# mgdesaix/WGSassign

Measured on AMD Instinct MI355X. Metric: EM SNP-updates/s (per-population update, n_call=100), higher is better.
Workload: dtype f64; 1 GPU; 1 GPU(s), SNP-sharded: synthetic Beagle 10000000 SNPs x 1000 ind, K=10, EM sweep; mode=exact, snps_per_gpu=10000000, gl_bytes_per_gpu=80000000000, comm_native_rccl=False, step=wgs_em_fit iteration (enqueued ahead of the host)

## Files before the change

### wgsassign_amd/csrc/codes.hip

```cpp
#include <chrono>
#include <cstdlib>
#include <cstring>

#include "common.h"

static double now_s() { return std::chrono::duration<double>(std::chrono::steady_clock::now().time_since_epoch()).count(); }

static void pool_join(wgs_beagle *b)
{
    if (b->pool_thread) {
        b->pool_thread->join();
        delete b->pool_thread;
        b->pool_thread = nullptr;
    }
}

static int pool_adopt(wgs_beagle *b)
{
    const int st = b->pool_state.load();
    if (st == 0) return b->pool ? 1 : -1;
    if (st == 1) return 0;
    pool_join(b);
    b->pool_state.store(0);
    if (st < 0) return -1;
// ... 53 lines not shown
    (void)hipFree(b->pool);
    b->pool = nullptr;
    b->pool_bytes = 0;
    return pool_request(b, want, want_small, grace_ms);
}

extern "C" int wgs_beagle_codes_wait(wgs_beagle *b, double *alloc_ms)
{
    WGS_REQUIRE(b, "null argument");
    if (alloc_ms) *alloc_ms = 0.0;
    if (b->pool_state.load() == 0) return 0;
    HIP_TRY(hipSetDevice(b->ctx->device));
    while (b->pool_state.load() == 1) std::this_thread::sleep_for(std::chrono::microseconds(100));
    (void)pool_adopt(b);
    if (alloc_ms) *alloc_ms = b->pool_alloc_ms;
    return 0;
}

void wgs_beagle_release_pool(wgs_beagle *b)
{
    if (!b) return;
    pool_join(b);
    if (b->pool_new) (void)hipFree(b->pool_new);
    b->pool_new = nullptr;
    b->pool_state.store(0);
    if (b->pool) (void)hipFree(b->pool);
    b->pool = nullptr;
    b->pool_bytes = 0;
}

void wgs_beagle_drop_codes(wgs_beagle *b)
{
    if (!b) return;
    if (wgs_codes *c = b->codes) {
        (void)hipSetDevice(b->ctx->device);
        (void)hipStreamSynchronize(b->ctx->stream);
        delete c;
    }
    b->codes = nullptr;
    b->codes_state = 0;
    b->plan = wgs_codes_plan();
    b->direct_sweeps = 0;
    ++b->codes_generation;
}

bool codes_switched_off()
{
    const char *env = getenv("WGSASSIGN_CODES");
    return env && env[0] == '0';
}

double wgs_em_codes_saving(double classes_per_slab, double cols, int lrows)
{
    const double saves = std::max(0.0, std::min(0.6, 1.0 - 2.2 * classes_per_slab / std::max(1.0, cols)));
    if (lrows <= 24) return saves;
    const double waves = std::max(1.0, std::min(13.0, floor(160.0 * 1024.0 / ((double)lrows * 512.0))));
    return std::max(0.0, 1.0 - (1.0 - saves) * pow(13.0 / waves, 0.8));
}

static int hist_quantile(const unsigned long long *h, double share)
{
    unsigned long long total = 0, run = 0;
    for (int i = 0; i < 256; ++i) total += h[i];
    if (!total) return 0;
    const double want = share * (double)total;
    for (int i = 0; i < 256; ++i) {
        run += h[i];
        if ((double)run >= want) return i;
    }
    return 255;
}

static double hist_mean(const unsigned long long *h)
{
    unsigned long long total = 0;
    double sum = 0.0;
    for (int i = 0; i < 256; ++i) total += h[i], sum += (double)i * (double)h[i];
    return total ? sum / (double)total : 0.0;
}

const wgs_codes_plan *wgs_beagle_codes_plan(wgs_beagle *b)
{
    if (!b) return nullptr;
    wgs_codes_plan &P = b->plan;
    if (P.state != 0) return &P;
    P = wgs_codes_plan();
    P.state = -1;
    if (hipSetDevice(b->ctx->device) != hipSuccess) return &P;
    const double t0 = now_s();
    wgs_codes tmpc;
    tmpc.slabs.resize(b->n_groups);
    for (int g = 0; g < b->n_groups; ++g) tmpc.slabs[g].nquads = (b->slabs[g].ncols + 3) / 4;
    void *tmp = nullptr;
    if (wgs_ctx_workspace_b(b->ctx, sizeof(SlabCodes) * b->n_groups, &tmp)) return &P;
    tmpc.d_slabs = reinterpret_cast<SlabCodes *>(tmp);
    if (hipMemcpy(tmpc.d_slabs, tmpc.slabs.data(), sizeof(SlabCodes) * b->n_groups, hipMemcpyHostToDevice) != hipSuccess) return &P;
    unsigned long long hg[256], hl[256];
    if (launch_class_sample(b, &tmpc, 4096, hg, hl, nullptr)) {
        (void)hipGetLastError();
        return &P;
    }
    P.mean_g = hist_mean(hg);
    P.mean_l = hist_mean(hl);
    const int g999 = hist_quantile(hg, 0.999), g99 = hist_quantile(hg, 0.99);
    const char *force = getenv("WGSASSIGN_CODES_TABLE");
    P.slots = g99 <= 44 ? 64 : (g99 <= 88 ? 128 : 256);
    if (force && (atoi(force) == 64 || atoi(force) == 128 || atoi(force) == 256)) P.slots = atoi(force);
// ... 202 lines not shown
```

### wgsassign_amd/csrc/common.h

```cpp
#pragma once
#include <hip/hip_runtime.h>
#include <stdint.h>

#include <atomic>
#include <chrono>
#include <thread>
#include <vector>

#include "../../include/wgsassign_hip.h"
#include "../../include/wgsassign_hip_debug.h"
#include "em_fit_ledger.h"

void wgs_set_error(const char *fmt, ...);

#ifdef WGS_TRACE_STALLS
#include <chrono>
#include <cstdio>
struct wgs_stall_probe {
    const char *what, *file;
    int line;
    std::chrono::steady_clock::time_point t0 = std::chrono::steady_clock::now();
    ~wgs_stall_probe() {
        const double ms = std::chrono::duration<double, std::milli>(std::chrono::steady_clock::now() - t0).count();
        if (ms >= WGS_TRACE_STALLS) fprintf(stderr, "[stall] %.1f ms in %s (%s:%d)\n", ms, what, file, line);
// ... 20 lines not shown
    } while (0)

extern std::atomic<long long> g_wgs_malloc_ns;
template <typename T>
static inline hipError_t wgs_malloc(T **p, size_t bytes)
{
    const auto t0 = std::chrono::steady_clock::now();
    const hipError_t e = hipMalloc(p, bytes);
    g_wgs_malloc_ns += std::chrono::duration_cast<std::chrono::nanoseconds>(std::chrono::steady_clock::now() - t0).count();
    return e;
}

#define WGS_REQUIRE(cond, ...)          \
    do {                                \
        if (!(cond)) {                  \
            wgs_set_error(__VA_ARGS__); \
            return 2;                   \
        }                               \
    } while (0)

template <typename F>
struct ScopeFail {
    F fn;
    bool armed = true;
    explicit ScopeFail(F f) : fn(f) {}
    ~ScopeFail() { if (armed) fn(); }
    void dismiss() { armed = false; }
};
template <typename F>
ScopeFail<F> on_failure(F f) { return ScopeFail<F>(f); }

struct wgs_ctx {
    int device = 0;
    hipStream_t stream = nullptr;
    void *pinned = nullptr;
    size_t pinned_bytes = 0;
    int cus = 0;
    void *ws = nullptr;
    size_t ws_bytes = 0;
    void *ws_b = nullptr;
    size_t ws_b_bytes = 0;
    bool log_table_ready = false;
    hipEvent_t ev0 = nullptr, ev1 = nullptr;
    float last_assign_ms = 0.0f;
    bool assign_ms_pending = false;
    std::atomic<int> allocs_in_flight{0};
    struct PoolBlock {
        void *p;
        size_t bytes;
        bool used;
    };
    std::vector<PoolBlock> pool;
    int64_t dyn_lds_base = -1;
    hipEvent_t enc_ev0 = nullptr, enc_ev1 = nullptr;
};
int wgs_ctx_workspace(wgs_ctx *ctx, size_t bytes, void **out);
hipError_t wgs_pool_malloc(wgs_ctx *ctx, void **p, size_t bytes);
void wgs_pool_free(wgs_ctx *ctx, void *p);
template <typename T>
static inline hipError_t wgs_pool_malloc(wgs_ctx *ctx, T **p, size_t bytes)
{
    return wgs_pool_malloc(ctx, reinterpret_cast<void **>(p), bytes);
}

struct Slab {
    float4 *base = nullptr;
    int32_t npairs = 0;
    int32_t ncols = 0;
    std::vector<int32_t> members;
    int32_t *d_members = nullptr;
};
static inline int64_t wgs_ntiles(int64_t m) { return (m + 63) / 64; }

#ifndef WGS_ENC_SLOTS
#define WGS_ENC_SLOTS 1024
#endif
constexpr int WGS_ENC_MIN_SNPS = WGS_ENC_SLOTS / 256;
constexpr int WGS_TILE_ROWS_BYTES = 64 / WGS_ENC_MIN_SNPS;
constexpr int WGS_BATCH_ROWS_CAP = 616;
struct SlabCodes {
    uint32_t *codes = nullptr;
    uint32_t *lcodes = nullptr;
    float2 *ldict = nullptr;
    uint8_t *tile_rows = nullptr;
    int32_t nquads = 0;
    int32_t quad0 = 0;
};
struct wgs_codes {
    void *pool = nullptr;
    int32_t snps_per_wave = 16;
    int32_t drows = 0;
    int32_t lrows = 0;
    int32_t cmax = 0;
    int32_t score_batch = 16;
    int32_t rows_batch = 0;
    int32_t total_quads = 0;
    float2 *dict = nullptr;
    uint8_t *ncls = nullptr;
    std::vector<SlabCodes> slabs;
    SlabCodes *d_slabs = nullptr;
    uint4 *wave_stats = nullptr;
    int64_t bytes = 0, local_bytes = 0;
    int64_t generation = 0;
    double build_ms = 0.0, kernel_ms = 0.0, sample_ms = 0.0, alloc_ms = 0.0, alloc_wait_ms = 0.0;
    double sum_ncls = 0.0;
    int64_t rich_snps = 0;
// ... 75 lines not shown
enum { WGS_LIVE_EM = 1, WGS_LIVE_SCORE = 2 };
void wgs_live_add(void *obj, int kind, void *parent, void *parent2 = nullptr);
bool wgs_live_remove(void *obj);
void wgs_live_destroy_children(void *parent);

int64_t wgs_hook(const char *name);

struct wgs_afset {
    wgs_ctx *ctx = nullptr;
    int64_t m = 0;
    int32_t K = 0;
    float *buf = nullptr;
};


struct FitDesc {
    const float4 *slab;
    const float *f_old;
    float *f_new;
    double *ssq;
    double *ssq_part;
    float *f_new2;
    double *ssq2;
    double *ssq_part2;
    int32_t fuse;
    int32_t npairs, ncols;
    int32_t skip;
    int32_t n_eff;
    const int32_t *state;
    const uint32_t *lcodes;
    const float2 *ldict;
    const uint8_t *tile_rows;
    int32_t nquads, lrows;
};
struct ChainJob {
    const float *a, *b;
    float carry_in;
};

struct FisherDesc {
    const float4 *slab;
    const float *th;
    float *f_out, *ne_out;
    int32_t npairs, ncols;
};
int launch_fisher_pop(wgs_ctx *ctx, const FisherDesc *d_descs, int32_t n_desc, int64_t m);
int launch_fisher_ind_sites(wgs_ctx *ctx, const float4 *slab, const int32_t *d_cols, const float *th, float *d_out, int64_t m,
                            int npairs, int count);
int launch_pairwise_mean(wgs_ctx *ctx, const float *d_rows, int count, int64_t m, int64_t divide_by, const int64_t *d_leaf_lo,
                         const int32_t *d_leaf_len, int nleaf, const int32_t *d_prog, int nprog, float *d_leaf_sums, const float *d_carry,
                         float *d_means);
int launch_em_sweep(wgs_ctx *ctx, const FitDesc *d_descs, int32_t n_fits, int64_t m, int mode);
int launch_em_coded(wgs_ctx *ctx, const FitDesc *d_descs, int32_t n_fits, int64_t m, int rows);
bool em_coded_usable(wgs_ctx *ctx);
int launch_em_coded_groups(wgs_ctx *ctx, const FitDesc *d_descs, const int32_t *d_groups, int32_t n_groups, int64_t m, int rows);
int em_fits_per_group(void);
int launch_em_sweep_groups(wgs_ctx *ctx, const FitDesc *d_descs, const int32_t *d_groups, int32_t n_groups, int64_t m, int mode);
int ssq_reduce_chunks(void);
int launch_ssq_reduce(wgs_ctx *ctx, const FitDesc *d_descs, int32_t n_fits, int64_t m, double *part2, int second = 0);
int launch_em_decide(wgs_ctx *ctx, const FitDesc *d_descs, int32_t n_fits, double lo, double hi);
int launch_rcp_error(wgs_ctx *ctx, int exponent, unsigned long long *d_max_bits);
int launch_div_check(wgs_ctx *ctx, unsigned long long seed, unsigned long long per_thread, unsigned long long *d_mismatch);
int launch_fill(wgs_ctx *ctx, float *p, int64_t count, float v);
int launch_clamp(wgs_ctx *ctx, float *p, int64_t count, float lo, float hi);
int launch_rmse_chain_serial(wgs_ctx *ctx, const float *a, const float *b, int64_t m, float carry_in, float *d_out);
size_t rmse_chain_workspace_bytes(int64_t m);
int launch_rmse_chain(wgs_ctx *ctx, const float *a, const float *b, int64_t m, float carry_in, float *d_out, void *work,
                      int *d_serial);
int launch_chain_set_carry(wgs_ctx *ctx, ChainJob *d_jobs, const float *d_carry, int n_jobs);
int launch_rmse_chain_batch(wgs_ctx *ctx, const ChainJob *d_jobs, int n_jobs, int64_t m, float *d_out, void *work, int *d_serial);
int launch_em_stream_add_sums(wgs_ctx *ctx, const double *d_window, double *d_total, int n);
int launch_em_stream_add_sums_above(wgs_ctx *ctx, const double *d_window, double *d_total, const int32_t *d_from, int t, int n);
int launch_em_stream_chain_load(wgs_ctx *ctx, ChainJob *d_jobs, const int32_t *d_cell, const float *d_table, int n_jobs);
int launch_em_stream_chain_store(wgs_ctx *ctx, const float *d_out, const int32_t *d_cell, float *d_table, int n_jobs);

struct AssignArgs {
    const float4 *slab;
    const int32_t *members;
    const float *const *colptr;
    const float *const *acol;
    double *out;
    int64_t m, site0;
    int32_t npairs, ncols, K, P;
    int32_t tiles_per_wave;
};
int launch_assign(wgs_ctx *ctx, const AssignArgs &a, int kb, int mode);
struct PartsSlab {
    const float4 *slab;
    const int32_t *members;
    int32_t npairs, ncols;
    int32_t block0;
};
int launch_parts_exact(wgs_ctx *ctx, const AssignArgs &a, const PartsSlab *d_slabs, int n_slabs, int total_blocks,
                       const float *d_carry, float *d_parts);

constexpr int WGS_BLOCK_TILES = 64;
struct ScoreSlab {
    const float4 *slab;
    const int32_t *members;
    int32_t npairs, ncols;
    int32_t pair0;
    int32_t npg;
    int32_t pg0;
    int32_t col_lo, col_hi;
};
struct ScoreArgs {
    const ScoreSlab *slabs;
// ... 61 lines not shown
```

### wgsassign_amd/csrc/em_api.hip

```cpp
#include <math.h>
#include <string.h>

#include <algorithm>
#include <chrono>
#include <string>

#include "common.h"
#include "em_state.h"
#include "em_stream_checks.h"

template <class Launch> static int em_launch_sliced(size_t units, size_t per_launch, Launch launch)
{
    for (size_t off = 0; off < units; off += per_launch)
        if (launch(off, (int)std::min(per_launch, units - off))) return 1;
    return 0;
}

extern "C" {



void wgs_em_destroy(wgs_em *em)
{
    if (!em || !wgs_live_remove(em)) return;
// ... 47 lines not shown
    em->pend_cur.assign(n_fits, 0);
    em->pend_prev.assign(n_fits, 1);
    em->active.assign(n_fits, 1);
    for (int j = 0; j < n_fits; ++j) {
        const int g = fit_group[j];
        if (g < 0 || g >= b->n_groups || b->slabs[g].ncols == 0) {
            wgs_set_error("fit %d: group %d is out of range or empty", j, g);
            return 2;
        }
        int skip = -1;
        if (fit_skip && fit_skip[j] >= 0) {
            const int i = fit_skip[j];
            if (i >= b->n || b->group_of[i] != g) {
                wgs_set_error("fit %d: left-out individual %d does not belong to group %d", j, i, g);
                return 2;
            }
            skip = b->col_of[i];
        }
        em->group[j] = g;
        em->skip_local[j] = skip;
        em->n_eff[j] = b->slabs[g].ncols - (skip >= 0 ? 1 : 0);
    }
    const size_t fbytes = (size_t)n_fits * b->m * sizeof(float);
    for (int i = 0; i < 2; ++i) {
        if (wgs_malloc(&em->fbuf[i], fbytes) != hipSuccess) {
            wgs_set_error("hipMalloc of %zu bytes for EM frequencies failed", fbytes);
            return 1;
        }
    }
    HIP_TRY(wgs_malloc(&em->d_ssq, sizeof(double) * n_fits));
    HIP_TRY(wgs_malloc(&em->d_part, sizeof(double) * (size_t)n_fits * wgs_ntiles(b->m)));
    HIP_TRY(wgs_malloc(&em->d_part2, sizeof(double) * (size_t)n_fits * ssq_reduce_chunks()));
    HIP_TRY(wgs_malloc(&em->d_carry, 2 * sizeof(float)));
    HIP_TRY(wgs_malloc(&em->d_chain_work, rmse_chain_workspace_bytes(b->m)));
    HIP_TRY(hipEventCreate(&em->ev0));
    HIP_TRY(hipEventCreate(&em->ev1));
    for (int i = 0; i < 2; ++i) {
        HIP_TRY(wgs_malloc(&em->d_descs[i], sizeof(FitDesc) * n_fits));
        HIP_TRY(hipHostMalloc(&em->h_descs[i], sizeof(FitDesc) * n_fits, hipHostMallocDefault));
        HIP_TRY(wgs_malloc(&em->d_groups[i], sizeof(int32_t) * 2 * n_fits));
        HIP_TRY(hipHostMalloc(&em->h_groups[i], sizeof(int32_t) * 2 * n_fits, hipHostMallocDefault));
    }
    if (launch_fill(b->ctx, em->fbuf[0], (int64_t)n_fits * b->m, 0.25f)) return 1;
    HIP_TRY(hipStreamSynchronize(b->ctx->stream));
    guard.dismiss();
    *out = em;
    return 0;
}


static double loo_codes_saving(const wgs_codes_plan *P, double cols)
{
    if (!P || P->state <= 0 || P->lrows == 0) return 0.0;
    return 1.0 - (1.7 * P->mean_l * 29.0 + 4.0 * cols + 250.0) / (25.9 * std::max(1.0, cols));
}

struct EmCodesModel {
    double direct_ms = 0.0, saves = 0.0, build_ms = 0.0;
    bool sampled = false;
    bool codable = false;
    bool pays = false;
};
static EmCodesModel em_codes_model(wgs_beagle *b, double swept, double cols, bool shared, bool sample)
{
    EmCodesModel M;
    if (shared) {
        constexpr double LOO_MS_PER_TERM = 7.6e-10;
        M.direct_ms = swept / 8.0 * LOO_MS_PER_TERM;
    } else {
        M.direct_ms = swept / 6.0e9;
        M.saves = wgs_em_codes_saving(4.6 * pow(std::max(1.0, cols), 0.25), cols, 24);
        M.build_ms = wgs_codes_build_ms_estimate(b, 64);
        M.codable = true;
        if (!sample) return M;
    }
    const wgs_codes_plan *P = wgs_beagle_codes_plan(b);
    M.sampled = true;
    M.codable = P && P->state > 0 && P->lrows > 0;
    if (!M.codable) {
        M.saves = 0.0;
        return M;
    }
    M.saves = shared ? std::max(0.0, loo_codes_saving(P, cols)) : wgs_em_codes_saving(P->mean_l, cols, P->lrows);
    M.build_ms = wgs_codes_build_ms_estimate(b, P->slots);
    return M;
}

static EmCodesModel em_codes_decide(wgs_beagle *b, double swept, double cols, bool shared, double ahead)
{
    const EmCodesModel T = em_codes_model(b, swept, cols, false, false);
    if (!shared && ahead * T.saves * T.direct_ms <= T.build_ms) return T;
    EmCodesModel M = em_codes_model(b, swept, cols, shared, true);
    M.pays = M.codable && ahead * M.saves * M.direct_ms > M.build_ms;
    return M;
}

static int env_int(const char *name, int unset) { const char *v = getenv(name); return v ? atoi(v) : unset; }

struct EmSwitches {
    bool codes = !codes_switched_off();
    bool loo_codes = env_int("WGSASSIGN_LOO_CODES", 1) != 0;
    int codes_min = env_int("WGSASSIGN_EM_CODES_MIN", 28);
    bool sweeps_set = getenv("WGSASSIGN_EM_CODES_SWEEPS") != nullptr;
    int sweeps_min = env_int("WGSASSIGN_EM_CODES_SWEEPS", 0);
    bool fuse = env_int("WGSASSIGN_EM_FUSE", 2) >= 2;
};

// ... 45 lines not shown
    const int64_t ntiles = wgs_ntiles(em->b->m);
    if (wgs_malloc(&em->fbuf[2], fbytes) != hipSuccess || wgs_malloc(&em->d_part_b, sizeof(double) * (size_t)em->n_fits * ntiles) != hipSuccess) {
        (void)hipGetLastError();
        if (em->fbuf[2]) (void)hipFree(em->fbuf[2]);
        em->fbuf[2] = nullptr;
        return false;
    }
    return true;
}

struct EmSweepPlan {
    std::vector<int32_t> order;
    bool shared = false;
    int fits_per_group = 1;
    wgs_codes *codes = nullptr;
    bool can_fuse = false;
    bool fusing = false;
    const std::vector<int32_t> *may_fuse = nullptr;
};

static EmSweepPlan em_plan_sweep(wgs_em *em, const std::vector<int32_t> &list, int sweeps_ahead, const std::vector<int32_t> *may_fuse,
                                 bool fuse_agreed, const EmSwitches &sw)
{
    wgs_beagle *b = em->b;
    EmSweepPlan p;
    double swept = 0.0, cols = 0.0;
    int fewest = INT32_MAX;
    std::vector<char> seen(b->n_groups, 0);
    for (int j : list) {
        const int g = em->group[j], ncols = b->slabs[g].ncols;
        p.shared = p.shared || seen[g];
        seen[g] = 1;
        swept += 8.0 * (double)ncols * (double)b->m;
        cols += (double)ncols;
        fewest = std::min(fewest, ncols);
    }
    cols /= (double)list.size();
    p.order = list;
    if (p.shared) std::stable_sort(p.order.begin(), p.order.end(), [&](int32_t x, int32_t y) { return em->group[x] < em->group[y]; });
    const bool worth = em->mode == WGS_MODE_EXACT && sw.codes && (!p.shared || sw.loo_codes) && fewest >= sw.codes_min &&
                       (!p.shared || sw.sweeps_set || loo_codes_saving(wgs_beagle_codes_plan(b), cols) > 0.03);
    const bool build = worth && em_codes_pay(em, swept, cols, sweeps_ahead, p.shared, sw);
    {
        WGS_STALL_SCOPE("wgs_beagle_codes from the sweep");
        p.codes = worth ? wgs_beagle_codes(b, build, false) : nullptr;
        if (p.codes && p.codes->lrows == 0 && p.codes->local_skipped && build) {
            const wgs_codes_plan keep = b->plan;
            wgs_beagle_drop_codes(b);
            b->plan = keep;
            p.codes = wgs_beagle_codes(b, true, false);
        }
    }
    WGS_STALL_SCOPE("the sweep's plan");
    if (p.codes && (p.codes->lrows == 0 || !em_coded_usable(b->ctx))) p.codes = nullptr;
    if (worth && !p.codes) ++b->direct_sweeps;
    if (p.codes && may_fuse && sw.fuse && !p.shared) {
        const bool wanted = std::any_of(p.order.begin(), p.order.end(), [&](int32_t j) { return (*may_fuse)[j] >= 2; });
        p.can_fuse = (em->fbuf[2] || wanted) && em_fuse_buffers(em);
        p.fusing = p.can_fuse && wanted && (fuse_agreed || wgs_hook("em_fuse_without_agreement") != 0);
    }
    p.may_fuse = may_fuse;
    if (p.shared) p.fits_per_group = p.codes ? 16 : em_fits_per_group();
    return p;
}

struct EmDescSlot {
    FitDesc *h, *d;
    int32_t *hg, *dg;
};
static EmDescSlot em_ring_slot(wgs_em *em, int slot) { return EmDescSlot{em->h_descs[slot], em->d_descs[slot], em->h_groups[slot], em->d_groups[slot]}; }

static int32_t em_write_descs(wgs_em *em, const EmSweepPlan &p, const EmDescSlot &slot, double *ssq, double *ssq_b, int32_t *state)
{
    const int64_t ntiles = wgs_ntiles(em->b->m);
    const int nb = em->fbuf[2] ? 3 : 2;
    for (size_t i = 0; i < p.order.size(); ++i) {
        const int j = p.order[i];
        const Slab &s = em->b->slabs[em->group[j]];
        FitDesc &d = slot.h[i];
        d.lcodes = p.codes ? p.codes->slabs[em->group[j]].lcodes : nullptr;
        d.ldict = p.codes ? p.codes->slabs[em->group[j]].ldict : nullptr;
        d.lrows = p.codes ? p.codes->lrows : 0;
        d.tile_rows = p.codes ? p.codes->slabs[em->group[j]].tile_rows : nullptr;
        d.nquads = p.codes ? p.codes->slabs[em->group[j]].nquads : 0;
        d.slab = s.base;
        const int fuse = p.fusing && (*p.may_fuse)[j] >= 2 ? 2 : 1;
        const EmBuffers first = em_rotate(em->cur[j], nb, 1), last = em_rotate(em->cur[j], nb, fuse);
        d.f_old = em_f(em, j, em->cur[j]);
        d.f_new = em_f(em, j, first.cur);
        d.f_new2 = em_f(em, j, last.cur);
        d.fuse = fuse;
        d.ssq = ssq + j;
        d.ssq2 = ssq_b ? ssq_b + j : d.ssq;
        d.ssq_part = em->d_part + (size_t)j * ntiles;
        d.ssq_part2 = fuse == 2 ? em->d_part_b + (size_t)j * ntiles : d.ssq_part;
        em->fuse_used[j] = (uint8_t)fuse;
        em->pend_cur[j] = last.cur;
        em->pend_prev[j] = last.prev;
        d.npairs = s.npairs;
        d.ncols = s.ncols;
        d.skip = em->skip_local[j];
        d.n_eff = em->n_eff[j];
        d.state = state ? state + j : nullptr;
    }
    int32_t n_groups = 0, *Hg = slot.hg;
    for (size_t i = 0; p.shared && i < p.order.size();) {
        size_t k = i + 1;
// ... 533 lines not shown
```

### wgsassign_amd/csrc/em_kernels.hip

```cpp
#include <type_traits>

#include "common.h"

namespace {

constexpr int WAVES = 4;
typedef float f4 __attribute__((ext_vector_type(4)));
typedef const f4 __attribute__((address_space(1))) *gf4_ptr;
typedef const float __attribute__((address_space(1))) *gf32_ptr;
typedef float __attribute__((address_space(1))) *gf32_wptr;
typedef const uint32_t __attribute__((address_space(1))) *gu32_ptr;
typedef const double __attribute__((address_space(1))) *gf64_ptr;

template <bool NT>
__device__ __forceinline__ f4 ldg(gf4_ptr p)
{
    if (NT) return __builtin_nontemporal_load(p);
    return *p;
}

struct SnpState {
    double fd, omf, fd2;
    float ff, omff, ff2;
};
// ... 264 lines not shown
}

typedef __attribute__((address_space(3))) uint32_t *lds_u32_ptr;
struct QTable {
    uint32_t lane4;
};
__device__ __forceinline__ QTable qtable_of(double *lds, int lane)
{
    (void)lds;
    QTable t;
    t.lane4 = (uint32_t)lane * 4u;
    return t;
}
template <int ROWS>
__device__ __forceinline__ void qtable_store(const QTable &t, int rank, double v)
{
    lds_u32_ptr p = (lds_u32_ptr)(uintptr_t)t.lane4;
    const unsigned long long bits = (unsigned long long)__double_as_longlong(v);
    p[rank * 64] = (uint32_t)bits;
    p[(ROWS + rank) * 64] = (uint32_t)(bits >> 32);
}
template <int ROWS, int H>
__device__ __forceinline__ double qtable_lookup(const QTable &t, uint32_t w)
{
    const uint32_t a = __builtin_amdgcn_perm(w, t.lane4, 0x0c0c0000u | ((4u + H) << 8));
    lds_u32_ptr p = (lds_u32_ptr)(uintptr_t)a;
    const uint32_t lo = p[0], hi = p[ROWS * 64];
    return __longlong_as_double((long long)(((unsigned long long)hi << 32) | lo));
}

template <int ILP, int ROWS>
__device__ __forceinline__ void coded_phase1_lane(const double (&r)[ROWS], const QTable &q, int nrows, float f_old)
{
    SnpState st;
    st.fd = (double)f_old;
    st.omf = 1.0 - st.fd;
    st.fd2 = 2.0 * st.fd;
#pragma unroll
    for (int r0 = 0; r0 < ROWS; r0 += ILP) {
        if (r0 < nrows) {
            double qv[ILP];
#pragma unroll
            for (int x = 0; x < ILP; ++x) {
                double raw = r[r0 + x];
                asm volatile("" : "+v"(raw));
                qv[x] = class_quotient(raw, st);
            }
#pragma unroll
            for (int x = 0; x < ILP; ++x) qtable_store<ROWS>(q, r0 + x, qv[x]);
        }
    }
}

template <int U, int ROWS>
__device__ __forceinline__ float coded_phase2(const QTable &q, gu32_ptr src, int nquads, int ncols, int skip, uint32_t (&cur)[U])
{
    const int last = nquads - 1;
    uint32_t nxt[U];
    float tmp = 0.0f;
    for (int q0 = 0; q0 < nquads; q0 += U) {
        if (q0 + U < nquads) {
#pragma unroll
            for (int u = 0; u < U; ++u) {
                const int qq = q0 + U + u;
                nxt[u] = src[(qq < last ? qq : last) * 64];
            }
        }
        double qv[U][4];
#pragma unroll
        for (int u = 0; u < U; ++u) {
            qv[u][0] = qtable_lookup<ROWS, 0>(q, cur[u]);
            qv[u][1] = qtable_lookup<ROWS, 1>(q, cur[u]);
            qv[u][2] = qtable_lookup<ROWS, 2>(q, cur[u]);
            qv[u][3] = qtable_lookup<ROWS, 3>(q, cur[u]);
        }
        const bool plain = 4 * (q0 + U) <= ncols && (skip < 4 * q0 || skip >= 4 * (q0 + U));
        if (plain) {
#pragma unroll
            for (int u = 0; u < U; ++u)
#pragma unroll
                for (int h = 0; h < 4; ++h) tmp = (float)__builtin_fma(0.5, qv[u][h], (double)tmp);
        } else {
#pragma unroll
            for (int u = 0; u < U; ++u)
#pragma unroll
                for (int h = 0; h < 4; ++h) {
                    const int col = 4 * (q0 + u) + h;
                    if (col < ncols && col != skip) tmp = (float)__builtin_fma(0.5, qv[u][h], (double)tmp);
                }
        }
#pragma unroll
        for (int u = 0; u < U; ++u) cur[u] = nxt[u];
    }
    return tmp;
}

#ifdef WGS_EM_STATS
__device__ unsigned long long g_em_stats[8];
#define EM_CLOCK(i) do { const unsigned long long now_ = clock64(); stat_[i] += now_ - mark_; mark_ = now_; } while (0)
#else
#define EM_CLOCK(i) do { } while (0)
#endif

template <int U, int ILP, int ROWS>
__device__ __forceinline__ float coded_iteration(const double (&r)[ROWS], const QTable &q, int nrows, gu32_ptr src, int nquads, int ncols, int skip, float f_old
#ifdef WGS_EM_STATS
                                                 , unsigned long long (&stat_)[8], unsigned long long &mark_
#endif
)
{
    const int last = nquads - 1;
    uint32_t cur[U];
#pragma unroll
    for (int u = 0; u < U; ++u) cur[u] = src[(u < last ? u : last) * 64];
    coded_phase1_lane<ILP, ROWS>(r, q, nrows, f_old);
#ifdef WGS_EM_STATS
    {
        const unsigned long long now_ = clock64();
        stat_[2] += now_ - mark_;
        mark_ = now_;
    }
#endif
    return coded_phase2<U, ROWS>(q, src, nquads, ncols, skip, cur);
}

template <int U, int ILP, int ROWS>
__global__ __launch_bounds__(64) void em_coded_kernel(const FitDesc *__restrict__ fits, int n_fits, int64_t m)
{
    extern __shared__ __align__(16) double qtab_all[];
    const unsigned xcd = blockIdx.x & 7u, j = blockIdx.x >> 3;
    const int fit = (int)(j % (unsigned)n_fits);
    const int64_t tile = (int64_t)(j / (unsigned)n_fits) * 8 + xcd;
    const FitDesc fd = fits[fit];
    if (fd.state && *fd.state != EM_ACTIVE) return;
    const int lane = threadIdx.x;
    const int64_t row0 = tile * 64;
    if (row0 >= m) return;
#ifdef WGS_EM_STATS
    unsigned long long stat_[8] = {0}, mark_ = clock64();
#endif
    const QTable q = qtable_of(qtab_all, lane);

    const int64_t my_row = row0 + lane;
    const int64_t my_row_c = my_row < m ? my_row : m - 1;
    float f_old = ((gf32_ptr)fd.f_old)[my_row_c];
    const int n_iter = fd.fuse == 2 ? 2 : 1;

    auto finish = [&](float tmp, int it) -> float {
        const float f_new = tmp / (float)fd.n_eff;
        double sq = 0.0;
        if (my_row < m) {
            ((gf32_wptr)(it ? fd.f_new2 : fd.f_new))[my_row] = f_new;
            const float d = f_new - f_old;
            sq = (double)(d * d);
        }
#pragma unroll
        for (int off = 32; off > 0; off >>= 1) sq += __shfl_down(sq, off, 64);
        if (lane == 0) (it ? fd.ssq_part2 : fd.ssq_part)[tile] = sq;
        return f_new;
    };

    const int nquads = fd.nquads;
    gu32_ptr src = (gu32_ptr)fd.lcodes + tile * nquads * 64 + lane;
    int nrows;
    {
        unsigned mx = 0;
#pragma unroll
        for (int x = 0; x < WGS_TILE_ROWS_BYTES / 8; ++x) {
            const unsigned long long w = reinterpret_cast<const unsigned long long *>(fd.tile_rows + tile * WGS_TILE_ROWS_BYTES)[x];
#pragma unroll
            for (int k = 0; k < 8; ++k) mx = max(mx, (unsigned)((w >> (8 * k)) & 255u));
        }
        nrows = (int)__builtin_amdgcn_readfirstlane((int)mx);
    }
    EM_CLOCK(0);
    if (nrows > ROWS || nrows > fd.lrows) {
        const int npairs = fd.npairs;
        gf4_ptr gl = (gf4_ptr)fd.slab + tile * npairs * 64 + lane;
        for (int it = 0; it < n_iter; ++it) {
            SnpState st;
            st.fd = (double)f_old;
            st.omf = 1.0 - st.fd;
            st.fd2 = 2.0 * st.fd;
            float tmp = 0.0f;
            bool ok = true;
            for (int p = 0; p < npairs; ++p) {
                const f4 v = gl[(int64_t)p * 64];
                if (2 * p < fd.ncols && 2 * p != fd.skip) term_exact<true>(v.x, v.y, st, tmp, ok);
                if (2 * p + 1 < fd.ncols && 2 * p + 1 != fd.skip) term_exact<true>(v.z, v.w, st, tmp, ok);
            }
            f_old = finish(tmp, it);
        }
        return;
    }
    double r[ROWS];
    {
        gf64_ptr drow = (gf64_ptr) reinterpret_cast<const double *>(fd.ldict) + tile * fd.lrows * 64 + lane;
#pragma unroll
        for (int g4 = 0; g4 < ROWS / 4; ++g4) {
            if (4 * g4 < nrows) {
#pragma unroll
                for (int u = 0; u < 4; ++u) r[4 * g4 + u] = drow[(int64_t)(4 * g4 + u) * 64];
            }
        }
    }
#ifdef WGS_EM_STATS
    {
        double any = 0.0;
#pragma unroll
        for (int x = 0; x < ROWS; x += 4)
            if (x < nrows) any += r[x];
        asm volatile("" : "+v"(any));
        EM_CLOCK(1);
    }
#endif
    for (int it = 0; it < n_iter; ++it) {
#ifdef WGS_EM_STATS
        const float tmp = coded_iteration<U, ILP, ROWS>(r, q, nrows, src, nquads, fd.ncols, fd.skip, f_old, stat_, mark_);
        EM_CLOCK(3);
        f_old = finish(tmp, it);
        EM_CLOCK(4);
#else
        const float tmp = coded_iteration<U, ILP, ROWS>(r, q, nrows, src, nquads, fd.ncols, fd.skip, f_old);
        f_old = finish(tmp, it);
#endif
    }
#ifdef WGS_EM_STATS
    if (lane == 0 && (blockIdx.x & 127u) < 8u) {
#pragma unroll
        for (int i = 0; i < 5; ++i) atomicAdd(&g_em_stats[i], stat_[i]);
        atomicAdd(&g_em_stats[5], (unsigned long long)n_iter);
        atomicAdd(&g_em_stats[6], 1ull);
    }
#endif
}

template <int U, int ILP, int ROWS>
__global__ __launch_bounds__(64) void em_coded_group_kernel(const FitDesc *__restrict__ fits, const int2 *__restrict__ groups, int n_groups, int64_t m)
{
    extern __shared__ __align__(16) double qtab_all[];
    const unsigned xcd = blockIdx.x & 7u, j = blockIdx.x >> 3;
    const int grp = (int)(j % (unsigned)n_groups);
    const int64_t tile = (int64_t)(j / (unsigned)n_groups) * 8 + xcd;
    const int lane = threadIdx.x;
    const int64_t row0 = tile * 64;
    if (row0 >= m) return;
    const int2 gd = groups[grp];
    const FitDesc *gf = fits + gd.x;
    const QTable q = qtable_of(qtab_all, lane);
    const int64_t my_row = row0 + lane;
    const int64_t my_row_c = my_row < m ? my_row : m - 1;
    const int nquads = gf[0].nquads, ncols = gf[0].ncols, lrows = gf[0].lrows;
    gu32_ptr src = (gu32_ptr)gf[0].lcodes + tile * nquads * 64 + lane;
    int nrows;
    {
        unsigned mx = 0;
#pragma unroll
        for (int x = 0; x < WGS_TILE_ROWS_BYTES / 8; ++x) {
            const unsigned long long w = reinterpret_cast<const unsigned long long *>(gf[0].tile_rows + tile * WGS_TILE_ROWS_BYTES)[x];
#pragma unroll
            for (int k = 0; k < 8; ++k) mx = max(mx, (unsigned)((w >> (8 * k)) & 255u));
        }
        nrows = (int)__builtin_amdgcn_readfirstlane((int)mx);
    }
    auto finish = [&](const FitDesc *fd, float tmp, float f_old) {
        const float f_new = tmp / (float)fd->n_eff;
        double sq = 0.0;
        if (my_row < m) {
            ((gf32_wptr)fd->f_new)[my_row] = f_new;
            const float d = f_new - f_old;
            sq = (double)(d * d);
        }
#pragma unroll
        for (int off = 32; off > 0; off >>= 1) sq += __shfl_down(sq, off, 64);
        if (lane == 0) fd->ssq_part[tile] = sq;
    };
    if (nrows > ROWS || nrows > lrows) {
        const int npairs = gf[0].npairs;
        gf4_ptr gl = (gf4_ptr)gf[0].slab + tile * npairs * 64 + lane;
        for (int f = 0; f < gd.y; ++f) {
            const FitDesc *fd = gf + f;
            if (fd->state && *fd->state != EM_ACTIVE) continue;
            const float f_old = ((gf32_ptr)fd->f_old)[my_row_c];
            const int skip = fd->skip;
            SnpState st;
            st.fd = (double)f_old;
            st.omf = 1.0 - st.fd;
            st.fd2 = 2.0 * st.fd;
            float tmp = 0.0f;
            bool ok = true;
            for (int p = 0; p < npairs; ++p) {
                const f4 v = gl[(int64_t)p * 64];
                if (2 * p < ncols && 2 * p != skip) term_exact<true>(v.x, v.y, st, tmp, ok);
                if (2 * p + 1 < ncols && 2 * p + 1 != skip) term_exact<true>(v.z, v.w, st, tmp, ok);
            }
            finish(fd, tmp, f_old);
        }
        return;
    }
    double r[ROWS];
    {
        gf64_ptr drow = (gf64_ptr) reinterpret_cast<const double *>(gf[0].ldict) + tile * lrows * 64 + lane;
#pragma unroll
        for (int g4 = 0; g4 < ROWS / 4; ++g4) {
            if (4 * g4 < nrows) {
#pragma unroll
                for (int u = 0; u < 4; ++u) r[4 * g4 + u] = drow[(int64_t)(4 * g4 + u) * 64];
            }
        }
    }
    float f_next = ((gf32_ptr)gf[0].f_old)[my_row_c];
    for (int f = 0; f < gd.y; ++f) {
        const FitDesc *fd = gf + f;
        const float f_old = f_next;
        if (f + 1 < gd.y) f_next = ((gf32_ptr)fd[1].f_old)[my_row_c];
        if (fd->state && *fd->state != EM_ACTIVE) continue;
#ifdef WGS_EM_STATS
        unsigned long long stat_[8] = {0}, mark_ = 0;
        const float tmp = coded_iteration<U, ILP, ROWS>(r, q, nrows, src, nquads, ncols, fd->skip, f_old, stat_, mark_);
#else
        const float tmp = coded_iteration<U, ILP, ROWS>(r, q, nrows, src, nquads, ncols, fd->skip, f_old);
#endif
        finish(fd, tmp, f_old);
    }
}

constexpr int RED_CHUNKS = 64;

__global__ __launch_bounds__(256) void ssq_reduce1_kernel(const FitDesc *__restrict__ fits, int64_t ntiles, double *__restrict__ part2, int second)
{
    __shared__ double red[256];
    const int fit = blockIdx.x / RED_CHUNKS, chunk = blockIdx.x % RED_CHUNKS;
    const FitDesc fd = fits[fit];
    const int64_t per = (ntiles + RED_CHUNKS - 1) / RED_CHUNKS;
    const int64_t t0 = chunk * per;
    int64_t t1 = t0 + per;
    if (t1 > ntiles) t1 = ntiles;
    double acc = 0.0;
    const double *part = second ? fd.ssq_part2 : fd.ssq_part;
    for (int64_t t = t0 + threadIdx.x; t < t1; t += 256) acc += part[t];
    red[threadIdx.x] = acc;
    __syncthreads();
    for (int w = 128; w > 0; w >>= 1) {
        if ((int)threadIdx.x < w) red[threadIdx.x] += red[threadIdx.x + w];
        __syncthreads();
    }
    if (threadIdx.x == 0) part2[blockIdx.x] = red[0];
}

__global__ __launch_bounds__(64) void ssq_reduce2_kernel(const FitDesc *__restrict__ fits, const double *__restrict__ part2, int second)
{
    double v = part2[blockIdx.x * RED_CHUNKS + threadIdx.x];
#pragma unroll
    for (int off = 32; off > 0; off >>= 1) v += __shfl_down(v, off, 64);
    if (threadIdx.x == 0) *(second ? fits[blockIdx.x].ssq2 : fits[blockIdx.x].ssq) = v;
}

__global__ void em_decide_kernel(const FitDesc *__restrict__ fits, int n_fits, double lo, double hi)
{
    const int j = blockIdx.x * blockDim.x + threadIdx.x;
    if (j >= n_fits) return;
    const FitDesc fd = fits[j];
    int32_t *st = const_cast<int32_t *>(fd.state);
    if (!st || *st != EM_ACTIVE) return;
    *st = em_decide(*fd.ssq, *fd.ssq2, fd.fuse, EmBand{lo, hi});
}

__global__ void fill_kernel(float *p, int64_t count, float v)
{
    int64_t i = (int64_t)blockIdx.x * blockDim.x + threadIdx.x;
    const int64_t stride = (int64_t)gridDim.x * blockDim.x;
    for (; i < count; i += stride) p[i] = v;
}

// ... 423 lines not shown
        const float s = (c & 0x3FFu) == 1 ? 0.0f : (p0 + p1) + p2;
        const double num = __builtin_fma(2.0, (double)p2, (double)p1), den = (double)s;
        const double q1 = div_exact(num, den), q2 = num / den;
        const bool same_bits = __double_as_longlong(q1) == __double_as_longlong(q2);
        const bool both_nan = q1 != q1 && q2 != q2;
        bad += !(same_bits || both_nan);
    }
    if (bad) atomicAdd(mismatch, bad);
}

__global__ void rcp_error_kernel(int exponent, unsigned long long *max_bits)
{
    const unsigned int mant = blockIdx.x * blockDim.x + threadIdx.x;
    if (mant >= (1u << 23)) return;
    const double den = __builtin_ldexp((double)__uint_as_float(0x3F800000u | mant), exponent);
    const double exact = 1.0 / den;
    const double err = __builtin_fabs(refined_rcp(den) - exact) / exact;
    atomicMax(max_bits, (unsigned long long)__double_as_longlong(err));
}

}

int launch_rcp_error(wgs_ctx *ctx, int exponent, unsigned long long *d_max_bits)
{
    hipLaunchKernelGGL(rcp_error_kernel, dim3((1u << 23) / 256), dim3(256), 0, ctx->stream, exponent, d_max_bits);
    HIP_TRY(hipGetLastError());
    return 0;
}

int launch_em_sweep(wgs_ctx *ctx, const FitDesc *d_descs, int32_t n_fits, int64_t m, int mode)
{
    if (n_fits <= 0 || m <= 0) return 0;
    const int64_t tiles = (m + 63) / 64;
    const int64_t blocks = (tiles + WAVES - 1) / WAVES * n_fits;
    WGS_REQUIRE(blocks < (1ll << 31), "em sweep: %lld workgroups exceed one launch; split the fit batch", (long long)blocks);
    dim3 grid((unsigned)blocks);
    if (mode == WGS_MODE_EXACT)
        hipLaunchKernelGGL((em_sweep_kernel<WGS_MODE_EXACT, 4>), grid, dim3(WAVES * 64), 0, ctx->stream, d_descs, n_fits, m);
    else
        hipLaunchKernelGGL((em_sweep_kernel<WGS_MODE_FAST, 4>), grid, dim3(WAVES * 64), 0, ctx->stream, d_descs, n_fits, m);
    HIP_TRY(hipGetLastError());
    return 0;
}

__global__ void dyn_lds_base_probe_kernel(uint32_t *out)
{
    extern __shared__ __align__(16) double probe_dyn[];
    if (threadIdx.x == 0) {
        probe_dyn[0] = 1.0;
        out[0] = (uint32_t)(uintptr_t)(__attribute__((address_space(3))) double *)probe_dyn;
    }
}

bool em_coded_usable(wgs_ctx *ctx)
{
    if (ctx->dyn_lds_base < 0) {
        uint32_t *d = nullptr, h = 0xffffffffu;
        if (hipMalloc(&d, sizeof(uint32_t)) == hipSuccess) {
            hipLaunchKernelGGL(dyn_lds_base_probe_kernel, dim3(1), dim3(64), 24 * 512, ctx->stream, d);
            if (hipMemcpyAsync(&h, d, sizeof(uint32_t), hipMemcpyDeviceToHost, ctx->stream) != hipSuccess ||
                hipStreamSynchronize(ctx->stream) != hipSuccess)
                h = 0xffffffffu;
            (void)hipFree(d);
        }
        (void)hipGetLastError();
        ctx->dyn_lds_base = (int64_t)h;
    }
    return ctx->dyn_lds_base == 0;
}

int launch_em_coded(wgs_ctx *ctx, const FitDesc *d_descs, int32_t n_fits, int64_t m, int rows)
{
    if (n_fits <= 0 || m <= 0) return 0;
    WGS_REQUIRE(rows >= 8 && rows <= 64 && rows % 8 == 0, "em sweep: %d table rows", rows);
    const int64_t tiles = (m + 63) / 64;
    const int64_t tgroups = (tiles + 7) / 8 * 8;
    const int64_t blocks = tgroups * n_fits;
    WGS_REQUIRE(blocks < (1ll << 31), "em sweep: %lld workgroups exceed one launch; split the fit batch", (long long)blocks);
    const size_t lds = (size_t)rows * 512 + (size_t)wgs_hook("em_coded_extra_lds");
#define WGS_EMC(RW) hipLaunchKernelGGL((em_coded_kernel<4, 2, RW>), dim3((unsigned)blocks), dim3(64), lds, ctx->stream, d_descs, n_fits, m)
    switch (rows) {
        case 8: WGS_EMC(8); break;
        case 16: WGS_EMC(16); break;
        case 24: WGS_EMC(24); break;
        case 32: WGS_EMC(32); break;
        case 40: WGS_EMC(40); break;
        case 48: WGS_EMC(48); break;
        case 56: WGS_EMC(56); break;
        default: WGS_EMC(64); break;
    }
#undef WGS_EMC
    HIP_TRY(hipGetLastError());
#ifdef WGS_EM_STATS
    {
        HIP_TRY(hipStreamSynchronize(ctx->stream));
        unsigned long long st[8] = {0}, zero[8] = {0};
        (void)hipMemcpyFromSymbol(st, HIP_SYMBOL(g_em_stats), sizeof st);
        (void)hipMemcpyToSymbol(HIP_SYMBOL(g_em_stats), zero, sizeof zero);
        const double w = st[6] ? (double)st[6] : 1.0;
        fprintf(stderr, "[em stats] %llu wavefronts, %.2f iterations each; cycles per wavefront: until the row count %.0f, until the dictionary rows %.0f, phase 1 %.0f, "
                "phase 2 %.0f, finishing %.0f\n", st[6], st[5] / w, st[0] / w, st[1] / w, st[2] / w, st[3] / w, st[4] / w);
    }
#endif
    return 0;
}

int launch_em_coded_groups(wgs_ctx *ctx, const FitDesc *d_descs, const int32_t *d_groups, int32_t n_groups, int64_t m, int rows)
{
    if (n_groups <= 0 || m <= 0) return 0;
    WGS_REQUIRE(rows >= 8 && rows <= 64 && rows % 8 == 0, "em sweep: %d table rows", rows);
    const int64_t tiles = (m + 63) / 64;
    const int64_t tgroups = (tiles + 7) / 8 * 8;
    const int64_t blocks = tgroups * n_groups;
    WGS_REQUIRE(blocks < (1ll << 31), "em sweep: %lld workgroups exceed one launch; split the fit batch", (long long)blocks);
    const int2 *g = reinterpret_cast<const int2 *>(d_groups);
    const size_t lds = (size_t)rows * 512;
// ... 230 lines not shown
```

Before: 7.397 billion SNP-updates/s.

## Prefetch coded quads through a register ring across EM iterations

Replaces the per-iteration cur/nxt double buffer in the coded EM kernel with a persistent register ring that is opened once before the row load and refilled as each slot is consumed. The next iteration's first code quads are then already in flight, removing a load-latency bubble at the start of each iteration and each fit. The code-saving cost-model constants are retuned so the coded path is chosen more often. The usability check now verifies that each kernel variant uses no static LDS and uses the context workspace instead of a fresh hipMalloc. The ring adds register pressure and an explicit vmcnt wait.

```diff
diff --git a/wgsassign_amd/csrc/codes.hip b/wgsassign_amd/csrc/codes.hip
--- a/wgsassign_amd/csrc/codes.hip
+++ b/wgsassign_amd/csrc/codes.hip
@@ -129,7 +129,7 @@
 
 double wgs_em_codes_saving(double classes_per_slab, double cols, int lrows)
 {
-    const double saves = std::max(0.0, std::min(0.6, 1.0 - 2.2 * classes_per_slab / std::max(1.0, cols)));
+    const double saves = std::max(0.0, std::min(0.63, 1.0 - 2.07 * classes_per_slab / std::max(1.0, cols)));
     if (lrows <= 24) return saves;
     const double waves = std::max(1.0, std::min(13.0, floor(160.0 * 1024.0 / ((double)lrows * 512.0))));
     return std::max(0.0, 1.0 - (1.0 - saves) * pow(13.0 / waves, 0.8));
diff --git a/wgsassign_amd/csrc/common.h b/wgsassign_amd/csrc/common.h
--- a/wgsassign_amd/csrc/common.h
+++ b/wgsassign_amd/csrc/common.h
@@ -96,6 +96,7 @@
     };
     std::vector<PoolBlock> pool;
     int64_t dyn_lds_base = -1;
+    uint32_t coded_static_seen = 0, coded_static_ok = 0;
     hipEvent_t enc_ev0 = nullptr, enc_ev1 = nullptr;
 };
 int wgs_ctx_workspace(wgs_ctx *ctx, size_t bytes, void **out);
@@ -277,7 +278,7 @@
                          float *d_means);
 int launch_em_sweep(wgs_ctx *ctx, const FitDesc *d_descs, int32_t n_fits, int64_t m, int mode);
 int launch_em_coded(wgs_ctx *ctx, const FitDesc *d_descs, int32_t n_fits, int64_t m, int rows);
-bool em_coded_usable(wgs_ctx *ctx);
+bool em_coded_usable(wgs_ctx *ctx, int rows, bool groups);
 int launch_em_coded_groups(wgs_ctx *ctx, const FitDesc *d_descs, const int32_t *d_groups, int32_t n_groups, int64_t m, int rows);
 int em_fits_per_group(void);
 int launch_em_sweep_groups(wgs_ctx *ctx, const FitDesc *d_descs, const int32_t *d_groups, int32_t n_groups, int64_t m, int mode);
diff --git a/wgsassign_amd/csrc/em_api.hip b/wgsassign_amd/csrc/em_api.hip
--- a/wgsassign_amd/csrc/em_api.hip
+++ b/wgsassign_amd/csrc/em_api.hip
@@ -123,7 +123,7 @@
 static double loo_codes_saving(const wgs_codes_plan *P, double cols)
 {
     if (!P || P->state <= 0 || P->lrows == 0) return 0.0;
-    return 1.0 - (1.7 * P->mean_l * 29.0 + 4.0 * cols + 250.0) / (25.9 * std::max(1.0, cols));
+    return 1.0 - (1.7 * P->mean_l * 29.0 + 4.0 * cols + 190.0) / (25.9 * std::max(1.0, cols));
 }
 
 struct EmCodesModel {
@@ -275,7 +275,7 @@
         }
     }
     WGS_STALL_SCOPE("the sweep's plan");
-    if (p.codes && (p.codes->lrows == 0 || !em_coded_usable(b->ctx))) p.codes = nullptr;
+    if (p.codes && (p.codes->lrows == 0 || !em_coded_usable(b->ctx, p.codes->lrows, p.shared))) p.codes = nullptr;
     if (worth && !p.codes) ++b->direct_sweeps;
     if (p.codes && may_fuse && sw.fuse && !p.shared) {
         const bool wanted = std::any_of(p.order.begin(), p.order.end(), [&](int32_t j) { return (*may_fuse)[j] >= 2; });
diff --git a/wgsassign_amd/csrc/em_kernels.hip b/wgsassign_amd/csrc/em_kernels.hip
--- a/wgsassign_amd/csrc/em_kernels.hip
+++ b/wgsassign_amd/csrc/em_kernels.hip
@@ -340,45 +340,69 @@
     }
 }
 
+constexpr int WAIT_VMCNT0 = 0x0F70;
+#ifndef WGS_EM_RING
+#define WGS_EM_RING 1
+#endif
+constexpr int EM_RING = WGS_EM_RING;
+
+template <int U>
+__device__ __forceinline__ void coded_ring_request(gu32_ptr base, uint32_t lane, int last, int q0, uint32_t (&buf)[U])
+{
+#pragma unroll
+    for (int u = 0; u < U; ++u) {
+        const int qq = q0 + u;
+        buf[u] = base[(uint32_t)(qq < last ? qq : last) * 64u + lane];
+    }
+}
+
+template <int U>
+__device__ __forceinline__ void coded_ring_open(gu32_ptr base, uint32_t lane, int nquads, uint32_t (&ring)[EM_RING + 1][U])
+{
+#pragma unroll
+    for (int s = 0; s <= EM_RING; ++s) coded_ring_request<U>(base, lane, nquads - 1, s * U, ring[s]);
+}
+
 template <int U, int ROWS>
-__device__ __forceinline__ float coded_phase2(const QTable &q, gu32_ptr src, int nquads, int ncols, int skip, uint32_t (&cur)[U])
+__device__ __forceinline__ float coded_phase2(const QTable &q, gu32_ptr base, uint32_t lane, int nquads, int ncols, int skip, uint32_t (&ring)[EM_RING + 1][U])
 {
     const int last = nquads - 1;
-    uint32_t nxt[U];
     float tmp = 0.0f;
-    for (int q0 = 0; q0 < nquads; q0 += U) {
-        if (q0 + U < nquads) {
-#pragma unroll
-            for (int u = 0; u < U; ++u) {
-                const int qq = q0 + U + u;
-                nxt[u] = src[(qq < last ? qq : last) * 64];
-            }
-        }
-        double qv[U][4];
-#pragma unroll
-        for (int u = 0; u < U; ++u) {
-            qv[u][0] = qtable_lookup<ROWS, 0>(q, cur[u]);
-            qv[u][1] = qtable_lookup<ROWS, 1>(q, cur[u]);
-            qv[u][2] = qtable_lookup<ROWS, 2>(q, cur[u]);
-            qv[u][3] = qtable_lookup<ROWS, 3>(q, cur[u]);
-        }
-        const bool plain = 4 * (q0 + U) <= ncols && (skip < 4 * q0 || skip >= 4 * (q0 + U));
-        if (plain) {
-#pragma unroll
-            for (int u = 0; u < U; ++u)
-#pragma unroll
-                for (int h = 0; h < 4; ++h) tmp = (float)__builtin_fma(0.5, qv[u][h], (double)tmp);
-        } else {
-#pragma unroll
-            for (int u = 0; u < U; ++u)
-#pragma unroll
-                for (int h = 0; h < 4; ++h) {
-                    const int col = 4 * (q0 + u) + h;
-                    if (col < ncols && col != skip) tmp = (float)__builtin_fma(0.5, qv[u][h], (double)tmp);
+    __builtin_amdgcn_s_waitcnt(WAIT_VMCNT0);
+    for (int qr = 0; qr < nquads; qr += (EM_RING + 1) * U) {
+#pragma unroll
+        for (int s = 0; s <= EM_RING; ++s) {
+            const int q0 = qr + s * U;
+            const bool live = s == 0 || q0 < nquads;
+            double qv[U][4];
+            if (live) {
+#pragma unroll
+                for (int u = 0; u < U; ++u) {
+                    qv[u][0] = qtable_lookup<ROWS, 0>(q, ring[s][u]);
+                    qv[u][1] = qtable_lookup<ROWS, 1>(q, ring[s][u]);
+                    qv[u][2] = qtable_lookup<ROWS, 2>(q, ring[s][u]);
+                    qv[u][3] = qtable_lookup<ROWS, 3>(q, ring[s][u]);
                 }
-        }
-#pragma unroll
-        for (int u = 0; u < U; ++u) cur[u] = nxt[u];
+            }
+            const int qn = q0 + (EM_RING + 1) * U;
+            coded_ring_request<U>(base, lane, last, qn < nquads ? qn : s * U, ring[s]);
+            if (!live) continue;
+            const bool plain = 4 * (q0 + U) <= ncols && (skip < 4 * q0 || skip >= 4 * (q0 + U));
+            if (plain) {
+#pragma unroll
+                for (int u = 0; u < U; ++u)
+#pragma unroll
+                    for (int h = 0; h < 4; ++h) tmp = (float)__builtin_fma(0.5, qv[u][h], (double)tmp);
+            } else {
+#pragma unroll
+                for (int u = 0; u < U; ++u)
+#pragma unroll
+                    for (int h = 0; h < 4; ++h) {
+                        const int col = 4 * (q0 + u) + h;
+                        if (col < ncols && col != skip) tmp = (float)__builtin_fma(0.5, qv[u][h], (double)tmp);
+                    }
+            }
+        }
     }
     return tmp;
 }
@@ -390,17 +414,22 @@
 #define EM_CLOCK(i) do { } while (0)
 #endif
 
+template <int ROWS>
+__device__ __forceinline__ void coded_rows_landed(double (&r)[ROWS], int nrows)
+{
+    (void)r;
+    (void)nrows;
+    __builtin_amdgcn_s_waitcnt(WAIT_VMCNT0);
+}
+
 template <int U, int ILP, int ROWS>
-__device__ __forceinline__ float coded_iteration(const double (&r)[ROWS], const QTable &q, int nrows, gu32_ptr src, int nquads, int ncols, int skip, float f_old
+__device__ __forceinline__ float coded_iteration(const double (&r)[ROWS], const QTable &q, int nrows, gu32_ptr base, uint32_t lane, uint32_t (&ring)[EM_RING + 1][U], int nquads,
+                                                 int ncols, int skip, float f_old
 #ifdef WGS_EM_STATS
                                                  , unsigned long long (&stat_)[8], unsigned long long &mark_
 #endif
 )
 {
-    const int last = nquads - 1;
-    uint32_t cur[U];
-#pragma unroll
-    for (int u = 0; u < U; ++u) cur[u] = src[(u < last ? u : last) * 64];
     coded_phase1_lane<ILP, ROWS>(r, q, nrows, f_old);
 #ifdef WGS_EM_STATS
     {
@@ -409,7 +438,7 @@
         mark_ = now_;
     }
 #endif
-    return coded_phase2<U, ROWS>(q, src, nquads, ncols, skip, cur);
+    return coded_phase2<U, ROWS>(q, base, lane, nquads, ncols, skip, ring);
 }
 
 template <int U, int ILP, int ROWS>
@@ -449,7 +478,9 @@
     };
 
     const int nquads = fd.nquads;
-    gu32_ptr src = (gu32_ptr)fd.lcodes + tile * nquads * 64 + lane;
+    gu32_ptr codes = (gu32_ptr)fd.lcodes + tile * nquads * 64;
+    uint32_t ring[EM_RING + 1][U];
+    coded_ring_open<U>(codes, (uint32_t)lane, nquads, ring);
     int nrows;
     {
         unsigned mx = 0;
@@ -492,24 +523,16 @@
             }
         }
     }
-#ifdef WGS_EM_STATS
-    {
-        double any = 0.0;
-#pragma unroll
-        for (int x = 0; x < ROWS; x += 4)
-            if (x < nrows) any += r[x];
-        asm volatile("" : "+v"(any));
-        EM_CLOCK(1);
-    }
-#endif
+    coded_rows_landed<ROWS>(r, nrows);
+    EM_CLOCK(1);
     for (int it = 0; it < n_iter; ++it) {
 #ifdef WGS_EM_STATS
-        const float tmp = coded_iteration<U, ILP, ROWS>(r, q, nrows, src, nquads, fd.ncols, fd.skip, f_old, stat_, mark_);
+        const float tmp = coded_iteration<U, ILP, ROWS>(r, q, nrows, codes, (uint32_t)lane, ring, nquads, fd.ncols, fd.skip, f_old, stat_, mark_);
         EM_CLOCK(3);
         f_old = finish(tmp, it);
         EM_CLOCK(4);
 #else
-        const float tmp = coded_iteration<U, ILP, ROWS>(r, q, nrows, src, nquads, fd.ncols, fd.skip, f_old);
+        const float tmp = coded_iteration<U, ILP, ROWS>(r, q, nrows, codes, (uint32_t)lane, ring, nquads, fd.ncols, fd.skip, f_old);
         f_old = finish(tmp, it);
 #endif
     }
@@ -539,7 +562,9 @@
     const int64_t my_row = row0 + lane;
     const int64_t my_row_c = my_row < m ? my_row : m - 1;
     const int nquads = gf[0].nquads, ncols = gf[0].ncols, lrows = gf[0].lrows;
-    gu32_ptr src = (gu32_ptr)gf[0].lcodes + tile * nquads * 64 + lane;
+    gu32_ptr codes = (gu32_ptr)gf[0].lcodes + tile * nquads * 64;
+    uint32_t ring[EM_RING + 1][U];
+    coded_ring_open<U>(codes, (uint32_t)lane, nquads, ring);
     int nrows;
     {
         unsigned mx = 0;
@@ -598,6 +623,7 @@
         }
     }
     float f_next = ((gf32_ptr)gf[0].f_old)[my_row_c];
+    coded_rows_landed<ROWS>(r, nrows);
     for (int f = 0; f < gd.y; ++f) {
         const FitDesc *fd = gf + f;
         const float f_old = f_next;
@@ -605,9 +631,9 @@
         if (fd->state && *fd->state != EM_ACTIVE) continue;
 #ifdef WGS_EM_STATS
         unsigned long long stat_[8] = {0}, mark_ = 0;
-        const float tmp = coded_iteration<U, ILP, ROWS>(r, q, nrows, src, nquads, ncols, fd->skip, f_old, stat_, mark_);
+        const float tmp = coded_iteration<U, ILP, ROWS>(r, q, nrows, codes, (uint32_t)lane, ring, nquads, ncols, fd->skip, f_old, stat_, mark_);
 #else
-        const float tmp = coded_iteration<U, ILP, ROWS>(r, q, nrows, src, nquads, ncols, fd->skip, f_old);
+        const float tmp = coded_iteration<U, ILP, ROWS>(r, q, nrows, codes, (uint32_t)lane, ring, nquads, ncols, fd->skip, f_old);
 #endif
         finish(fd, tmp, f_old);
     }
@@ -1137,16 +1163,49 @@
     }
 }
 
-bool em_coded_usable(wgs_ctx *ctx)
-{
+template <typename F>
+static int64_t coded_static_lds_of(F *kernel)
+{
+    hipFuncAttributes attr;
+    if (hipFuncGetAttributes(&attr, reinterpret_cast<const void *>(kernel)) != hipSuccess) {
+        (void)hipGetLastError();
+        return -1;
+    }
+    return (int64_t)attr.sharedSizeBytes;
+}
+static int64_t coded_static_lds(int rows, bool groups)
+{
+#define WGS_EMS(RW) (groups ? coded_static_lds_of(em_coded_group_kernel<4, 2, RW>) : coded_static_lds_of(em_coded_kernel<4, 2, RW>))
+    switch (rows) {
+        case 8: return WGS_EMS(8);
+        case 16: return WGS_EMS(16);
+        case 24: return WGS_EMS(24);
+        case 32: return WGS_EMS(32);
+        case 40: return WGS_EMS(40);
+        case 48: return WGS_EMS(48);
+        case 56: return WGS_EMS(56);
+        default: return WGS_EMS(64);
+    }
+#undef WGS_EMS
+}
+
+bool em_coded_usable(wgs_ctx *ctx, int rows, bool groups)
+{
+    const int slot = (rows >= 8 && rows <= 64 ? rows / 8 - 1 : 7) + (groups ? 8 : 0);
+    if (!(ctx->coded_static_seen >> slot & 1u)) {
+        ctx->coded_static_seen |= 1u << slot;
+        if (coded_static_lds(rows, groups) == 0) ctx->coded_static_ok |= 1u << slot;
+    }
+    if (!(ctx->coded_static_ok >> slot & 1u)) return false;
     if (ctx->dyn_lds_base < 0) {
-        uint32_t *d = nullptr, h = 0xffffffffu;
-        if (hipMalloc(&d, sizeof(uint32_t)) == hipSuccess) {
+        uint32_t h = 0xffffffffu;
+        void *ws = nullptr;
+        if (wgs_ctx_workspace(ctx, 256, &ws) == 0) {
+            uint32_t *d = reinterpret_cast<uint32_t *>(ws);
             hipLaunchKernelGGL(dyn_lds_base_probe_kernel, dim3(1), dim3(64), 24 * 512, ctx->stream, d);
             if (hipMemcpyAsync(&h, d, sizeof(uint32_t), hipMemcpyDeviceToHost, ctx->stream) != hipSuccess ||
                 hipStreamSynchronize(ctx->stream) != hipSuccess)
                 h = 0xffffffffu;
-            (void)hipFree(d);
         }
         (void)hipGetLastError();
         ctx->dyn_lds_base = (int64_t)h;
```

Result: no change. 7.407 billion SNP-updates/s, median of 2 (+0.1%).
